# benjjneb/dada2

Measured on AMD Instinct MI355X. Metric: unique reads denoised/sec (dada() wall-clock), higher is better.
Workload: dtype int32 DP + f64 lambda/p-value

## Files before the change

dada2_amd/csrc/driver.cpp:

```cpp
#include <fcntl.h>
#include <sys/file.h>
#include <unistd.h>

#include <algorithm>
#include <atomic>
#include <chrono>
#include <condition_variable>
#include <exception>
#include <mutex>
#include <cmath>
#include <cstdarg>
#include <cstdio>
#include <cstring>
#include <ctime>
#include <memory>
#include <thread>
#include <unordered_map>

#include "engine.h"
#include "hostpar.h"
#include "knobs.h"
#include "ppois.h"

namespace d2 {
// ... 1544 lines not shown
    if (knobs().v2_summary) fprintf(stderr, "[v3] entry barrier failed after %ld blocks: continuing on the launch chains\n", v2_cons);
  }
  bool v3_block_ready() const { return *(volatile int32_t *)&v2_hblk.p[v2_cons % RING2].seq == (int32_t)(v2_cons + 1); }
  long v3_ended() const { return (long)*(volatile int32_t *)(v3_hflags.p + 16); }
  std::vector<EnqRec> v3_rec;
  void v3_enqueue(bool first) {
    const auto t_enq = clk::now();
    hipStream_t stq = s->stream;
    EnqRec rec{-1, -1, !first};
    if (!first) {
      rec.ev_screen = ev_begin(EV_SCREEN, profile_all, true);
      launch2_screen_multi(E2, stq);
      ev_end(rec.ev_screen);
      launch2_batch_lists(E2, stq);
      const NwBatch nb{&v2_ctl.p->nalign, v2_blistn.p, v2_blist.p, v2_ctl.p->acentre, &v2_ctl.p->abuf, E2.C.Npad, v2_bretry.p, v2_bretryn.p, v2_retrytot.p, &v2_ctl.p->fast_off};
      launch_gapless_batch(s->D, nb, ap, s->d_err.p, v2_lamB.p, v2_hamB.p, &v2_ctl.p->state, stq);
      rec.ev_nw = ev_begin(EV_NW, profile_all, true);
      launch_nw_ad(s->D, -1, nullptr, nullptr, nullptr, 0, nullptr, nullptr, ap, s->d_err.p, v2_lamB.p, v2_hamB.p, nullptr, 0, 0, nullptr, stq,
                   &v2_ctl.p->state, &nb);
      ev_end(rec.ev_nw);
    }
    const int ev = ev_begin(EV_TAIL, profile_all);
    Eng2 Ek = E2;
    if (!profile_all) Ek.ktime = nullptr;
    Ek.pf_plan = (v3_overlap && (active_runs(s->device).load() <= 1 || knobs().v3_overlap == 1)) ? 1 : 0;
    launch3_tail(Ek, v3_grid, first, (int)(v3_enq + 1), s->h_reads[bi[0].center], stq);
    ev_end(ev);
    v3_rec.push_back(rec);
    v3_enq++;
    st.ms_enqueue += ms_since(t_enq);
  }

  void v3_pf_enqueue(long k) {
    const auto t_enq = clk::now();
    hipStream_t st2 = s->cmp;
    Ctl2 *pc = v3_pfctl.p;
    *(volatile int32_t *)(v3_hflags.p + 40 + (k & 7)) = 0;
    launch2_pf_gate(E2P, (int)k, v3_hflags.p + 32, v3_hflags.p + 40 + (k & 7), st2);
    launch2_pf_tables(E2P, st2);
    int ev = ev_begin(EV_PF_SCREEN, profile_all, false, false, st2);
    launch2_screen_multi(E2P, st2);
    ev_end(ev);
    launch2_batch_lists(E2P, st2);
    const NwBatch nb{&pc->nalign, v3_pf_blistn.p, v3_pf_blist.p, pc->acentre, &pc->abuf, E2.C.Npad, v3_pf_bretry.p, v3_pf_bretryn.p, v2_retrytot.p, &pc->fast_off};
    launch_gapless_batch(S2, nb, ap, s->d_err.p, v2_lamB.p, v2_hamB.p, &pc->state, st2);
    ev = ev_begin(EV_PF_NW, profile_all, false, false, st2);
    launch_nw_ad(S2, -1, nullptr, nullptr, nullptr, 0, nullptr, nullptr, ap, s->d_err.p, v2_lamB.p, v2_hamB.p, nullptr, 0, 0, nullptr, st2,
                 &pc->state, &nb);
    ev_end(ev);
    launch2_pf_done(E2P, st2);
    D2_HIP(hipEventRecord(v3_pf_ev[k & 3], st2));
    v3_pf_launched = std::max(v3_pf_launched, k);
    v3_pf_chains++;
    st.ms_enqueue += ms_since(t_enq);
  }
  int v3_pf_gate_result(long k) const { return (int)*(volatile int32_t *)(v3_hflags.p + 40 + (k & 7)); }
  int32_t v3_pf_stat[4] = {0, 0, 0, 0};
  void v3_pf_totals() {
    PfSync ps;
    D2_HIP(hipMemcpy(&ps, v3_pfsync.p, sizeof ps, hipMemcpyDeviceToHost));
// ... 191 lines not shown
    if (lite) st.lite_chains++;
    v2_enqrec.push_back(rec);
    v2_enq++;
    st.ms_enqueue += ms_since(t_enq);
  }
  void v2_round_launches(int nlev, bool with_compare, bool store, EnqRec *recp, bool lite = false) {
    hipStream_t stq = s->stream;
    EnqRec rec{-1, -1, with_compare};
    const Eng2 &E2 = lite ? this->E2L : this->E2;
    if (with_compare && !lite) {
      rec.ev_screen = ev_begin(EV_SCREEN, profile_all, true);
      launch2_screen_multi(E2, stq);
      ev_end(rec.ev_screen);
      launch2_batch_lists(E2, stq);
      const NwBatch nb{&v2_ctl.p->nalign, v2_blistn.p, v2_blist.p, v2_ctl.p->acentre, &v2_ctl.p->abuf, E2.C.Npad, v2_bretry.p, v2_bretryn.p, v2_retrytot.p, &v2_ctl.p->fast_off};
      launch_gapless_batch(s->D, nb, ap, s->d_err.p, v2_lamB.p, v2_hamB.p, &v2_ctl.p->state, stq);
      rec.ev_nw = ev_begin(EV_NW, profile_all, true);
      launch_nw_ad(s->D, -1, nullptr, nullptr, nullptr, 0, nullptr, nullptr, ap, s->d_err.p, v2_lamB.p, v2_hamB.p, nullptr, 0, 0, nullptr, stq,
                   &v2_ctl.p->state, &nb);
      ev_end(rec.ev_nw);
    }
    int ev = ev_begin(EV_SHUFFLE, profile_all && nlev > 0);
    for (int l = 0; l < nlev; l++) launch2_shuffle(E2, l, store && l == 0, stq);
    ev_end(ev);
    ev = ev_begin(EV_PVAL, profile_all);
    launch2_eval(E2, nlev, s->h_reads[bi[0].center], stq);
    ev_end(ev);
    if (recp) *recp = rec;
  }

  const Round2Out &v2_wait_block() {
// ... 1380 lines not shown
```

dada2_amd/csrc/engine.h:

```cpp
#pragma once
#include <cstddef>
#include <cstdint>
#include <string>
#include <vector>

#include <hip/hip_runtime.h>

#include "../../include/dada2hip.h"

namespace d2 {

constexpr int KMER_SIZE = 5;
constexpr int NKMER = 1024;
constexpr int RANK_SAT = 63;
constexpr int MAX_SHUFFLE = 10;
constexpr int SEQLEN = 9999;
constexpr double TAIL_APPROX_CUTOFF = 1e-7;

enum : uint8_t { CLS_SKIP = 0, CLS_SHROUD = 1, CLS_GAPLESS = 2, CLS_NW = 3 };

struct DeviceError {
  int code;
  std::string msg;
};
// ... 167 lines not shown
               double *d_lambda, uint32_t *d_ham, uint16_t *d_view, int LV, int view_by_chunk, uint8_t *d_moves,
               int moves_stride, int32_t *d_nmoves, hipStream_t st, const int32_t *d_pair_centre = nullptr);

struct NwBatch {
  const int32_t *on;
  const int32_t *n;
  const int32_t *list;
  const int32_t *centre;
  const int32_t *bbuf;
  size_t stride;
  int32_t *retry_list = nullptr;
  int32_t *retry_n = nullptr;
  unsigned long long *fast_ctl = nullptr;
  const int32_t *fast_off = nullptr;
};
void launch_gapless_batch(const SampleDev &S, const NwBatch &b, const AlignParams &ap, const double *d_err, double *d_lambda,
                          uint32_t *d_ham, const int32_t *d_stop_dev, hipStream_t st);
void launch_nw_ad(const SampleDev &S, int centre, const int32_t *d_chunk_centre, const int32_t *d_work,
                  const int32_t *d_nwork, int nwork_host, const int32_t *d_gl_work, const int32_t *d_gl_nwork,
                  const AlignParams &ap, const double *d_err, double *d_lambda, uint32_t *d_ham, uint16_t *d_view, int LV,
                  int view_by_chunk, const int32_t *d_centre_dev, hipStream_t st, const int32_t *d_stop_dev = nullptr,
                  const NwBatch *batch = nullptr);
int nw_ad_apw(const SampleDev &S, const AlignParams &ap);
size_t nw_ad_lds_bytes(const SampleDev &S, const AlignParams &ap);
void launch_nw_ad_lr(const SampleDev &S, const int32_t *d_chunk_centre, const int32_t *d_work, int nwork, const AlignParams &ap,
                     const double *d_err, int allow_one_off, int max_shift, int32_t *d_out, hipStream_t st);
size_t nw_ad_lr_lds_bytes(const SampleDev &S, const AlignParams &ap);

bool nw_adw_ok(const SampleDev &S, const AlignParams &ap);
size_t nw_adw_ptr_words_per_wave(const SampleDev &S, const AlignParams &ap);
int nw_adw_waves(const SampleDev &S, const AlignParams &ap, int nwork);
size_t nw_adw_lds_bytes(const SampleDev &S, const AlignParams &ap);
// ... 307 lines not shown
```

dada2_amd/csrc/kernels.hip:

```cpp
#include <atomic>
#include <cstring>

#include "engine.h"
#include "gcn.h"
#include "knobs.h"
#include "rounds_common.h"
#include "ppois.h"

namespace d2 {

static std::atomic<uint64_t> g_ledger[LEDGER_WORDS];
void ledger_note(int bit) { g_ledger[bit >> 6].fetch_or((uint64_t)1 << (bit & 63), std::memory_order_relaxed); }
void ledger_read(uint64_t *out, bool clear) {
  for (int w = 0; w < LEDGER_WORDS; w++)
    out[w] = clear ? g_ledger[w].exchange(0, std::memory_order_relaxed) : g_ledger[w].load(std::memory_order_relaxed);
}
static std::atomic<int32_t> g_nw_trips{0};
void nw_trips_note(int trips) {
  int32_t cur = g_nw_trips.load(std::memory_order_relaxed);
  while (cur < trips && !g_nw_trips.compare_exchange_weak(cur, trips, std::memory_order_relaxed)) {}
}
int nw_trips_read(bool clear) { return clear ? g_nw_trips.exchange(0, std::memory_order_relaxed) : g_nw_trips.load(std::memory_order_relaxed); }

static __device__ __forceinline__ uint32_t base_at(const uint32_t *__restrict__ row, int p) {
// ... 302 lines not shown
    ham[r] = h;
  }
}

void launch_gapless(const SampleDev &S, int centre, const int32_t *d_chunk_centre, const int32_t *d_work,
                    const int32_t *d_nwork, int nwork_host, const AlignParams &ap, const double *d_err,
                    double *d_lambda, uint32_t *d_ham, uint16_t *d_view, int LV, int view_by_chunk, hipStream_t st) {
  int maxwork = d_nwork ? S.N : nwork_host;
  if (maxwork <= 0) return;
  int grid = std::min((maxwork + 255) / 256, 2048);
  ledger_note(LEDGER_GAPLESS);
  hipLaunchKernelGGL(k_gapless, dim3(grid), dim3(256), (size_t)16 * ap.ncol * sizeof(double), st, S, centre,
                     d_chunk_centre, d_work, d_nwork, nwork_host, ap, d_err, d_lambda, d_ham, d_view, LV, view_by_chunk);
}

__global__ __launch_bounds__(256) void k_gapless_batch(SampleDev S, NwBatch b, AlignParams ap, const double *__restrict__ err,
                                                       double *__restrict__ lam, uint32_t *__restrict__ ham, const int32_t *__restrict__ stop_dev) {
  if (stop_dev && *stop_dev != 0) return;
  const int nb = *b.on;
  if (nb <= 0) return;
  int wk[KB_MAX + 1];
  wk[0] = 0;
#pragma unroll
  for (int k = 0; k < KB_MAX; k++) wk[k + 1] = wk[k] + (k < nb ? (b.n[KB_MAX + k] + 63) / 64 : 0);
  if ((int)blockIdx.x * 4 >= wk[KB_MAX]) return;
  extern __shared__ double s_err[];
  for (int i = threadIdx.x; i < 16 * ap.ncol; i += blockDim.x) s_err[i] = err[i];
  __syncthreads();
  const int lane = threadIdx.x & 63, gwave = blockIdx.x * 4 + (threadIdx.x >> 6), nwaves = gridDim.x * 4;
  for (int w = gwave; w < wk[KB_MAX]; w += nwaves) {
    int k = 0, w0 = 0;
#pragma unroll
    for (int q = 1; q < KB_MAX; q++) if (w >= wk[q]) { k = q; w0 = wk[q]; }
    const int idx = (w - w0) * 64 + lane;
    if (idx >= b.n[KB_MAX + k]) continue;
    const int r = b.list[(size_t)(KB_MAX + k) * b.stride + idx], c = b.centre[k];
    const uint32_t *crow = S.seq2 + (size_t)c * S.W2, *rrow = S.seq2 + (size_t)r * S.W2;
    const uint8_t *qrow = S.qual + (size_t)r * S.LQ;
    const int L1 = S.len[c], L2 = S.len[r];
    double l = 1.0;
    uint32_t h = 0, cw = 0, rw = 0, qw = 0;
    for (int p = 0; p < L2; p++) {
      if ((p & 15) == 0) { rw = rrow[p >> 4]; cw = p < L1 ? crow[p >> 4] : 0; }
      if ((p & 3) == 0) qw = *(const uint32_t *)(qrow + p);
      const uint32_t rb = (rw >> ((p & 15) << 1)) & 3u, q = ap.use_quals ? ((qw >> ((p & 3) << 3)) & 255u) : 0u;
      uint32_t t = 5u * rb;
      if (p < L1) {
        const uint32_t cb = (cw >> ((p & 15) << 1)) & 3u;
        t = 4u * cb + rb;
        h += (cb != rb);
      }
      l = l * s_err[t * ap.ncol + q];
    }
    const size_t o = ((size_t)*b.bbuf * KB_MAX + k) * b.stride + r;
    lam[o] = l;
    ham[o] = h;
  }
}
void launch_gapless_batch(const SampleDev &S, const NwBatch &b, const AlignParams &ap, const double *d_err, double *d_lambda,
                          uint32_t *d_ham, const int32_t *d_stop_dev, hipStream_t st) {
  const int grid = std::min((S.N + 255) / 256 + KB_MAX, 2048);
  ledger_note(LEDGER_GAPLESS + 1);
  hipLaunchKernelGGL(k_gapless_batch, dim3(grid), dim3(256), (size_t)16 * ap.ncol * sizeof(double), st, S, b, ap, d_err, d_lambda, d_ham,
                     d_stop_dev);
}

struct NwArgs {
  SampleDev S;
  int centre;
  const int32_t *centre_dev;
  const int32_t *chunk_centre;
  const int32_t *pair_centre;
  const int32_t *work;
  const int32_t *nwork_dev;
  int nwork_host;
  AlignParams ap;
  const double *err;
  uint32_t *ptr_scr;
  uint32_t *t_scr;
// ... 4 lines not shown
  uint16_t *view;
  int LV;
  int view_by_chunk;
  uint8_t *moves;
  int moves_stride;
  int32_t *nmoves;
  const int32_t *stop_dev;
  int32_t *lr_out;
  int lr_one_off, lr_max_shift;
  const int32_t *batch_on;
  const int32_t *batch_n;
  const int32_t *batch_list;
  const int32_t *batch_centre;
  const int32_t *batch_bbuf;
  size_t batch_stride;
  int32_t *retry_list;
  int32_t *retry_n;
  unsigned long long *fast_ctl;
  const int32_t *fast_off;
  const int32_t *alt_list;
  const int32_t *alt_n;
};

template <int NPW>
static __device__ __forceinline__ void nw_traceback_lambda(const NwArgs &a, const double *s_err, int lane, int idx,
                                                           bool active, int r, int c, int L1, int L2, int lband,
                                                           const uint32_t *ptr, uint32_t *tsc, int npw_rt, int chunk) {
  const SampleDev &S = a.S;
  const size_t vr = a.view_by_chunk ? (size_t)chunk : (size_t)r;
  const uint32_t *crow = S.seq2 + (size_t)c * S.W2, *rrow = S.seq2 + (size_t)r * S.W2;
// ... 461 lines not shown
__global__ __launch_bounds__(256, 4) void k_nw_ad(NwArgs a, const int32_t *__restrict__ gl_work, const int32_t *__restrict__ gl_nwork_dev,
                                               AdGeom G) {
  static_assert(!FAST || (DEF && !LR && !HOMO), "the pointer-free pass exists for the default scores of the denoising path");
  constexpr int APW = 64 / GL;
  extern __shared__ __attribute__((aligned(16))) double s_dyn[];
  double *s_err = s_dyn;
  const int nerr = 16 * a.ap.ncol;
  const bool batch = a.batch_on != nullptr;
  int bk[KB_MAX + 1];
  {
    if (a.stop_dev && *a.stop_dev != 0) return;
    bk[0] = 0;
    if (batch) {
      const int nb = *a.batch_on;
      if (nb <= 0) return;
      if (a.fast_off) {
        const bool off = *a.fast_off != 0;
        if (FAST) {
          if (off) return;
          if (blockIdx.x == 0 && threadIdx.x == 0) {
            unsigned long long tot = 0;
            for (int k = 0; k < KB_MAX; k++) tot += k < nb ? (unsigned long long)a.batch_n[k] : 0ull;
            atomicAdd(&a.fast_ctl[1], tot);
          }
        } else if (off && a.alt_list) { a.batch_list = a.alt_list; a.batch_n = a.alt_n; }
      }
#pragma unroll
      for (int k = 0; k < KB_MAX; k++) bk[k + 1] = bk[k] + (k < nb ? (a.batch_n[k] + 4 * APW - 1) / (4 * APW) : 0);
      if ((int)blockIdx.x >= bk[KB_MAX]) return;
    } else {
      const int n_all = (a.nwork_dev ? *a.nwork_dev : a.nwork_host) + (gl_work ? *gl_nwork_dev : 0);
      if ((int)blockIdx.x * 4 * APW >= n_all) return;
      if (a.centre_dev && *a.centre_dev < 0) return;
    }
  }
  for (int i = threadIdx.x; i < nerr; i += blockDim.x) s_err[i] = a.err[i];
  const int wib = threadIdx.x >> 6, lane = threadIdx.x & 63;
  const bool ghost = lane / GL >= APW;
  const int al = ghost ? APW - 1 : lane / GL, g = ghost ? GL : lane % GL;
  uint8_t *blk0 = (uint8_t *)(s_dyn + nerr);
// ... 12 lines not shown
      for (int p = threadIdx.x; p < Lc; p += 256) cwd[p] = ad_base_word<HOMO>(S.seq2 + (size_t)cv * S.W2, Lc, p);
    }
  }
  __syncthreads();
  const int gwave = blockIdx.x * 4 + wib;
  uint32_t *pg = S.ad_ptr + (size_t)gwave * S.ad_wpw;
  int n_nw = batch ? 0 : (a.nwork_dev ? *a.nwork_dev : a.nwork_host);
  const int n_gl = batch ? 0 : (gl_work ? *gl_nwork_dev : 0);
  int nwork = n_nw + n_gl;
  const int SENT = a.ap.sentinel, MATCH = a.ap.match, MISMATCH = a.ap.mismatch, GAP = a.ap.gap, B = a.ap.band, HGAP = a.ap.homo_gap;
  const int centre_v = batch ? 0 : (a.centre_dev ? *a.centre_dev : a.centre);
  if (centre_v < 0 && !a.chunk_centre) return;
  const int32_t *wl = a.work, *gll = gl_work;
  size_t out_off = 0;
  int kcur = -1;
  for (int it = blockIdx.x;; it += gridDim.x) {
    int chunk, c;
    if (batch) {
      if (it >= bk[KB_MAX]) break;
      int k = 0, b0 = 0;
#pragma unroll
      for (int q = 1; q < KB_MAX; q++) if (it >= bk[q]) { k = q; b0 = bk[q]; }
      c = a.batch_centre[k];
      if (k != kcur) {
        __syncthreads();
        const int Lc = S.len[c];
        for (int p = threadIdx.x; p < Lc; p += 256) cwd[p] = ad_base_word<HOMO>(S.seq2 + (size_t)c * S.W2, Lc, p);
        __syncthreads();
        kcur = k;
        wl = a.batch_list + (size_t)k * a.batch_stride; gll = a.batch_list + (size_t)(KB_MAX + k) * a.batch_stride;
        n_nw = a.batch_n[k]; nwork = n_nw;
// ... 20 lines not shown
      for (int p = g; p < L2; p += GL) rwd[p] = ad_base_word<HOMO>(S.seq2 + (size_t)r * S.W2, L2, p);
    if (LR && !ghost)
      for (int w = g; w < 3 * G.bmw; w += GL) bm[w] = 0;
    int ecol = 0;
    const uint8_t *qrow = S.qual + (size_t)r * S.LQ;
    const size_t vr = a.view_by_chunk ? (size_t)chunk : (size_t)r;
    if (a.view && active && !ghost)
      for (int p = g; p < L1; p += GL) a.view[vr * a.LV + p] = 0;
    int Tmax = T;
#pragma unroll
    for (int o = 32; o >= 1; o >>= 1) Tmax = max(Tmax, __shfl_xor(Tmax, o, 64));
    const int dbg = a.moves_stride;
    Tmax = gcn_readfirstlane(Tmax);
    const int org = (EDGE ? 0 : 2) + (lband & 1), lbo = lband + org;
    uint32_t acc0 = ~0u, acc1 = ~0u, ep0 = 3u, ep1 = 3u;
    if (Tmax >= 0 && !(dbg & 1)) {
      int d0 = SENT, d1 = SENT;
      uint32_t pw = 0;
      int i = (lbo >> 1) - g, j = -i;
      uint32_t cb = cwd[i - 1], rb = rwd[j - 1];
      const bool g_first = g == 0, g_last = ghost || g == GL - 1;
      const bool kok0 = !ghost && 2 * g >= org && 2 * g < W + org, kok1 = !ghost && 2 * g + 1 >= org && 2 * g + 1 < W + org;
      constexpr int KUP = ADK_GAP + (int)AD_UP - (int)AD_DIAG, KLEFT = ADK_GAP + (int)AD_LEFT - (int)AD_DIAG;
      const int gs0 = DEF ? (kok0 ? KUP : ADK_BIG) : (kok0 ? GAP : AD_OOB), gs1 = DEF ? (kok1 ? KLEFT : ADK_BIG) : (kok1 ? GAP : AD_OOB);
      const int gn0 = DEF ? ((EDGE && g_first) || !kok0 ? ADK_BIG : KLEFT) : gs0, gn1 = DEF ? ((EDGE && g_last) || !kok1 ? ADK_BIG : KUP) : gs1;
      if (DEF) { d0 = ADK_BIG + (int)AD_DIAG; d1 = ADK_BIG + (int)AD_DIAG; }
      int tA = (lband > rband ? lband : rband) + 2, tB = min(2 * L1 - lband, 2 * L2 - rband);
      if (T < 0) { tA = 0; tB = 0x3FFFFFFF; }
#pragma unroll
      for (int o = 32; o >= 1; o >>= 1) { tA = max(tA, __shfl_xor(tA, o, 64)); tB = min(tB, __shfl_xor(tB, o, 64)); }
      tA = gcn_readfirstlane(tA);
      tB = gcn_readfirstlane(tB);
#define AD_FLUSH(TT) { if (!FAST) { pg[(size_t)((TT) >> 4) * 64 + lane] = pw; pw = 0; } }
#define AD_STEP(PARV, LEANV, VNEXT, FS, KOK, GS)                                                                                   \
  {                                                                                                                             \
    if (FAST) ad_step_k<GL, PARV, LEANV, EDGE, true>(d0, d1, i, j, cb, rb, (PARV) ? acc1 : acc0, (VNEXT), (FS), g_first, g_last, (KOK), (GS), (PARV) ? gn1 : gn0, L1, L2, (PARV) ? &ep1 : &ep0); \
    else if (DEF) ad_step_k<GL, PARV, LEANV, EDGE>(d0, d1, i, j, cb, rb, pw, (VNEXT), (FS), g_first, g_last, (KOK), (GS), (PARV) ? gn1 : gn0, L1, L2); \
    else ad_step<GL, PARV, DEF, LEANV, EDGE, HOMO>(d0, d1, i, j, cb, rb, pw, (VNEXT), (FS), g_first, g_last, (KOK), (GS), L1, L2, SENT, MATCH, MISMATCH, GAP, HGAP); \
  }
#define AD_FULL_STEP(TT)                                                                                                        \
  {                                                                                                                             \
    if (((TT) & 1) == 0) AD_STEP(0, false, rwd[j], ((TT) & 15) << 1, kok0, gs0)                                                 \
    else AD_STEP(1, false, cwd[i], ((TT) & 15) << 1, kok1, gs1)                                                                 \
    if (((TT) & 15) == 15) AD_FLUSH(TT)                                                                                         \
  }
#define AD_LEAN_PAIR(TT)                                                                                                        \
  {                                                                                                                             \
    AD_STEP(0, true, rwd[j], ((TT) & 15) << 1, kok0, gs0)                                                                       \
    AD_STEP(1, true, cwd[i], (((TT) + 1) & 15) << 1, kok1, gs1)                                                                 \
    if ((((TT) + 1) & 15) == 15) AD_FLUSH((TT) + 1)                                                                             \
  }
// ... 6 lines not shown
        __builtin_memcpy(rwv, rwd + j, 32);
        __builtin_memcpy(cwv, cwd + i, 32);
#pragma unroll
        for (int u = 0; u < 8; u++) {
          AD_STEP(0, true, rwv[u], 4 * u, kok0, gs0)
          AD_STEP(1, true, cwv[u], 4 * u + 2, kok1, gs1)
        }
        AD_FLUSH(t)
      }
      for (; t + 2 <= tB && t + 1 <= Tmax; t += 2) AD_LEAN_PAIR(t)
      for (; t <= Tmax; t++) AD_FULL_STEP(t)
#undef AD_LEAN_PAIR
#undef AD_FULL_STEP
#undef AD_STEP
#undef AD_FLUSH
      if (!FAST && ((t - 1) & 15) != 15) pg[(size_t)((t - 1) >> 4) * 64 + lane] = pw >> (2 * (15 - ((t - 1) & 15)));
    }
    int fres = 0, fk = 0, fm = 0, fdir = -1;
    if (FAST) {
      fk = L2 - L1 + lbo;
      if (T < 0) fres = 2;
      for (int itw = 0; itw <= 2 * GL + 1; itw++) {
        if (__all(fres != 0)) break;
        const bool inband = fk >= org && fk < W + org;
        const int src = al * GL + (inband ? (fk >> 1) : 0);
        const uint32_t e0 = (uint32_t)__shfl((int)ep0, src, 64), e1 = (uint32_t)__shfl((int)ep1, src, 64);
        const uint32_t a0 = (uint32_t)__shfl((int)acc0, src, 64), a1 = (uint32_t)__shfl((int)acc1, src, 64);
        if (fres != 0) continue;
        const uint32_t pe = (fk & 1) ? e1 : e0, whole = (((fk & 1) ? a1 : a0) >> 1) & 1u;
        if (!inband || pe > AD_DIAG) fres = 2;
        else if (pe == AD_DIAG) fres = whole ? 1 : 2;
        else if (fdir < 0 || (int)pe == fdir) { fdir = (int)pe; fm++; fk += pe == AD_UP ? 1 : -1; }
        else fres = 2;
      }
      if (fres == 0) fres = 2;
    }
    int ti = L1, tj = L2;
    bool done = !active || (dbg & 2);
    uint32_t h = 0;
    int guard = L1 + L2 + 2;
    while (true) {
      int nruns = 0;
      uint32_t last = 0;
      auto push = [&](int lo, int n, int dl) {
        if (last) {
          const int llo = last & 4095, ln = (last >> 12) & 4095, ldl = (int)(last >> 24);
          if (ldl == dl && lo + n == llo) { last = (uint32_t)lo | ((uint32_t)(ln + n) << 12) | ((uint32_t)dl << 24); return; }
          runs[nruns++] = last;
        }
        last = (uint32_t)lo | ((uint32_t)n << 12) | ((uint32_t)dl << 24);
      };
      const bool lead = g == 0 && !ghost;
      if (lead && !done && gapless) {
        const int n = L1 < L2 ? L1 : L2;
        runs[nruns++] = 0u | ((uint32_t)n << 12) | (128u << 24);
        if (L2 > n) runs[nruns++] = (uint32_t)n | ((uint32_t)(L2 - n) << 12) | (255u << 24);
        done = true;
      }
      if (FAST && lead && !done) {
        if (fres == 1) {
          const int dd = fk - lbo;
          const int n = dd >= 0 ? min(L1, L2 - dd) : min(L1 + dd, L2);
          if (fdir == (int)AD_LEFT && fm > 0) runs[nruns++] = (uint32_t)(L2 - fm) | ((uint32_t)fm << 12) | (255u << 24);
          if (n > 0) runs[nruns++] = (uint32_t)(dd >= 0 ? dd : 0) | ((uint32_t)n << 12) | ((uint32_t)(128 - dd) << 24);
          if (dd > 0) runs[nruns++] = 0u | ((uint32_t)dd << 12) | (255u << 24);
        } else if (active && !gapless) {
          const int q = atomicAdd(&a.retry_n[kcur], 1);
          a.retry_list[(size_t)kcur * a.batch_stride + q] = r;
          if (a.fast_ctl) atomicAdd(&a.fast_ctl[0], 1ull);
        }
        done = true; ti = 0; tj = 0;
      }
      const int gl0 = al * GL;
      if (!FAST)
      for (;;) {
        const bool act = lead && !done && (ti > 0 || tj > 0) && nruns < AD_RCAP - 2 && guard > 0;
        if (!__any(act)) break;
        bool gapmove = false;
        const int gact = __shfl((int)act, gl0, 64);
        const int tt = __shfl(ti + tj, gl0, 64), col = __shfl((tj - ti + lbo) >> 1, gl0, 64);
        const int f0 = tt & 15, widx = (tt >> 4) - g;
        uint32_t word = 0xAAAAAAAAu;
        if (gact && !ghost && widx >= 0) word = pg[(size_t)widx * 64 + gl0 + col];
        const int ftop = g == 0 ? f0 : 14 + (f0 & 1);
        const uint32_t x = word ^ 0xAAAAAAAAu;
        uint32_t nz = (x | (x >> 1)) & 0x55555555u;
        nz &= (f0 & 1) ? 0x44444444u : 0x11111111u;
        nz &= (ftop == 15) ? 0xFFFFFFFFu : ((1u << ((ftop + 1) << 1)) - 1u);
        const bool st = nz != 0;
// ... 83 lines not shown
      if (__all(done)) break;
    }
    if (LR) {
      gcn_wave_sync();
      if (g == 0 && !ghost && active)
        bimera_lr_bits(bm, bm + G.bmw, bm + 2 * G.bmw, ecol, a.lr_one_off, a.lr_max_shift, a.lr_out + (size_t)idx * 5);
      continue;
    }
    if (g == 0 && !ghost) runs[0] = 0;
    gcn_wave_sync();
    if (!ghost && h) atomicAdd(&runs[0], h);
    gcn_wave_sync();
    h = runs[0];
    const long long fid = ((long long)it * 4 + wib) * APW + al;
    const bool offload = S.ad_foff != nullptr && fid < (long long)S.ad_fcap && !(dbg & 8);
    if (FAST && fres != 1) continue;
    if (offload) {
      if (active && !ghost) {
        uint16_t *fo = S.ad_foff + (size_t)fid * S.ad_fstride;
        for (int pj = g; pj < L2; pj += GL) fo[pj] = (uint16_t)rwd[pj];
        if (g == 0) {
          AdDesc d;
          d.dest = (long long)(out_off + r); d.L2 = L2; d.pad = 0;
          S.ad_desc[fid] = d;
          a.ham[out_off + r] = h;
        }
      }
    } else
    if (g == 0 && active && !(dbg & 8)) {
      const char *eb = (const char *)s_err;
      auto fetch8 = [&](int pj, double (&f)[8]) __attribute__((always_inline)) {
// ... 15 lines not shown
          for (int k = 0; k < 8; k++) f[k] = n[k];
        }
#pragma unroll
        for (int k = 0; k < 8; k++) l = l * f[k];
      }
      for (; pj < L2; pj++) l = l * *(const double *)(eb + rwd[pj]);
      a.lam[out_off + r] = l;
      a.ham[out_off + r] = h;
    }
  }
}

__global__ __launch_bounds__(256) void k_ad_product(const uint16_t *__restrict__ foff, int stride, AdDesc *__restrict__ desc, int nscan,
                                                    const double *__restrict__ err, int nerr, double *__restrict__ lam,
                                                    const int32_t *__restrict__ stop_dev, const int32_t *__restrict__ batch_on,
                                                    const int32_t *__restrict__ batch_n, int slots_per_slice,
                                                    const int32_t *__restrict__ fast_off = nullptr, const int32_t *__restrict__ alt_n = nullptr) {
  extern __shared__ double s_err[];
  if (stop_dev && *stop_dev != 0) return;
  if (fast_off && alt_n && *fast_off != 0) batch_n = alt_n;
  if (batch_on) {
    const int nb = *batch_on;
    if (nb <= 0) return;
    int slices = 0;
    for (int k = 0; k < KB_MAX; k++) slices += k < nb ? (batch_n[k] + slots_per_slice - 1) / slots_per_slice : 0;
    nscan = min(nscan, slices * slots_per_slice);
  }
  if ((int)(blockIdx.x * blockDim.x) >= nscan) return;
  for (int i = threadIdx.x; i < nerr; i += blockDim.x) s_err[i] = err[i];
  __syncthreads();
  const char *eb = (const char *)s_err;
  for (int id = blockIdx.x * blockDim.x + threadIdx.x; id < nscan; id += gridDim.x * blockDim.x) {
    const AdDesc d = desc[id];
    if (d.dest < 0) continue;
    desc[id].dest = -1;
// ... 26 lines not shown
  a.S = S; a.centre = centre; a.chunk_centre = d_chunk_centre; a.work = d_work; a.nwork_dev = d_nwork;
  a.nwork_host = nwork_host; a.ap = ap; a.err = d_err; a.lam = d_lambda; a.ham = d_ham;
  a.view = d_view; a.LV = LV; a.view_by_chunk = view_by_chunk; a.centre_dev = d_centre_dev; a.stop_dev = d_stop_dev;
#ifdef DADA2HIP_PROFILING
  a.moves_stride = knobs().ad_debug;
#endif
  if (batch) {
    a.batch_on = batch->on; a.batch_n = batch->n; a.batch_list = batch->list; a.batch_centre = batch->centre; a.batch_bbuf = batch->bbuf;
    a.batch_stride = batch->stride;
  }
  const AdGeom G = ad_geom(ap.band, S.maxlen, S.minlen, d_chunk_centre ? 0 : 1);
  const size_t lds = (size_t)16 * ap.ncol * 8 + (size_t)G.block_bytes;
  int waves = (std::max(maxwork, 1) + G.APW - 1) / G.APW;
  if (d_gl_work || batch) waves = (S.N + G.APW - 1) / G.APW;
  int grid = std::max(1, std::min((waves + 3) / 4, std::min(256 * 8, S.ad_waves / 4)));
  const bool homo = ap.endsfree && ap.homo_gap != ap.gap;
  const bool def = !homo && ap.match == 5 && ap.mismatch == -4 && ap.gap == -8 && ap.sentinel == -32760;
  const bool fast = batch && def && batch->retry_list && batch->retry_n && batch->fast_off && knobs().ad_fast != 0 && a.moves_stride == 0;
  auto set_lds = [&](const void *fn, std::atomic<size_t> (&done)[64]) {
    int dev_ = 0;
    (void)hipGetDevice(&dev_);
    std::atomic<size_t> &d = done[dev_ & 63];
    if (lds > d.load(std::memory_order_acquire)) {
      (void)hipFuncSetAttribute(fn, hipFuncAttributeMaxDynamicSharedMemorySize, (int)lds);
      d.store(lds, std::memory_order_release);
    }
  };
#define D2_LAUNCH_AD(GLV, DEFV, EDGEV, HOMOV, FASTV)                                                                     \
  do {                                                                                                                   \
    static std::atomic<size_t> attr_set[64];                                                                             \
    set_lds((const void *)k_nw_ad<GLV, DEFV, EDGEV, false, HOMOV, FASTV>, attr_set);                                     \
    ledger_note(LEDGER_AD + 8 * (GLV == 21 ? 0 : GLV == 32 ? 1 : 2) + 4 * (EDGEV ? 1 : 0) + (FASTV ? 3 : HOMOV ? 2 : DEFV ? 0 : 1)); \
    hipLaunchKernelGGL((k_nw_ad<GLV, DEFV, EDGEV, false, HOMOV, FASTV>), dim3(grid), dim3(256), lds, st, a, d_gl_work, d_gl_nwork, G);  \
  } while (0)
#define D2_LAUNCH_AD2(GLV, FASTV)                                                                                        \
  do {                                                                                                                   \
    if (FASTV) { if (G.edge) D2_LAUNCH_AD(GLV, true, true, false, FASTV); else D2_LAUNCH_AD(GLV, true, false, false, FASTV); } \
    else if (homo) { if (G.edge) D2_LAUNCH_AD(GLV, false, true, true, false); else D2_LAUNCH_AD(GLV, false, false, true, false); } \
    else if (def) { if (G.edge) D2_LAUNCH_AD(GLV, true, true, false, false); else D2_LAUNCH_AD(GLV, true, false, false, false); } \
    else { if (G.edge) D2_LAUNCH_AD(GLV, false, true, false, false); else D2_LAUNCH_AD(GLV, false, false, false, false); }   \
  } while (0)
  auto product = [&](const int32_t *list_n, const int32_t *foff = nullptr, const int32_t *alt_n = nullptr) {
    if (!(S.ad_foff && a.moves_stride == 0)) return;
    const int nerr = 16 * ap.ncol;
    long long bound = batch ? (long long)S.ad_fcap : (long long)((maxwork + (d_gl_work ? S.N : 0) + 4 * G.APW - 1) / (4 * G.APW) + 1) * 4 * G.APW;
    const int nscan = (int)std::min<long long>(bound, S.ad_fcap);
    const int pgrid = std::max(1, std::min((nscan + 255) / 256, 2048));
    hipLaunchKernelGGL(k_ad_product, dim3(pgrid), dim3(256), (size_t)nerr * 8, st, (const uint16_t *)S.ad_foff, (int)S.ad_fstride, S.ad_desc, nscan, d_err, nerr,
                       d_lambda, d_stop_dev, batch ? batch->on : nullptr, list_n, 4 * G.APW, foff, alt_n);
  };
  if (fast) {
    a.retry_list = batch->retry_list; a.retry_n = batch->retry_n; a.fast_ctl = batch->fast_ctl; a.fast_off = batch->fast_off;
    if (G.GL == 21) D2_LAUNCH_AD2(21, true);
    else if (G.GL == 32) D2_LAUNCH_AD2(32, true);
    else D2_LAUNCH_AD2(64, true);
    product(batch->n);
    a.alt_list = a.batch_list; a.alt_n = a.batch_n;
    a.batch_list = batch->retry_list; a.batch_n = batch->retry_n;
    a.retry_list = nullptr; a.retry_n = nullptr;
  }
  if (G.GL == 21) D2_LAUNCH_AD2(21, false);
  else if (G.GL == 32) D2_LAUNCH_AD2(32, false);
  else D2_LAUNCH_AD2(64, false);
#undef D2_LAUNCH_AD2
#undef D2_LAUNCH_AD
  if (fast) product(batch->retry_n, batch->fast_off, batch->n);
  else product(batch ? batch->n : nullptr);
}

void launch_nw_ad_lr(const SampleDev &S, const int32_t *d_chunk_centre, const int32_t *d_work, int nwork, const AlignParams &ap,
                     const double *d_err, int allow_one_off, int max_shift, int32_t *d_out, hipStream_t st) {
  if (nwork <= 0) return;
  NwArgs a;
  memset(&a, 0, sizeof a);
  a.S = S; a.chunk_centre = d_chunk_centre; a.work = d_work; a.nwork_host = nwork; a.ap = ap; a.err = d_err;
  a.lr_out = d_out; a.lr_one_off = allow_one_off; a.lr_max_shift = max_shift;
  const AdGeom G = ad_geom(ap.band, S.maxlen, S.minlen, 0, 1);
  const size_t lds = (size_t)16 * ap.ncol * 8 + (size_t)G.block_bytes;
  const int waves = (nwork + G.APW - 1) / G.APW;
  const int grid = std::max(1, std::min((waves + 3) / 4, std::min(256 * 8, S.ad_waves / 4)));
  const bool def = ap.match == 5 && ap.mismatch == -4 && ap.gap == -8 && ap.sentinel == -32760;
#define D2_LAUNCH_LR(GLV, DEFV, EDGEV)                                                                                   \
// ... 1144 lines not shown
```

Baseline: 7.380 million.

## Fuse gapless batch into NW kernel blocks and resweep fast-path failures in-kernel

Removes the separate gapless-batch kernel launch and runs its work in extra blocks appended to the k_nw_ad grid, selected by block index. The FAST variant now resweeps failing alignments in place with full pointer recording instead of pushing them to a retry list. The product kernel is also launched once at the end instead of twice. This cuts kernel launches and queue gaps in the compare chain, at the cost of a larger grid, mixed block roles, and more register and code pressure in the NW kernel.

```diff
diff --git a/dada2_amd/csrc/driver.cpp b/dada2_amd/csrc/driver.cpp
--- a/dada2_amd/csrc/driver.cpp
+++ b/dada2_amd/csrc/driver.cpp
@@ -1582,7 +1582,6 @@
       ev_end(rec.ev_screen);
       launch2_batch_lists(E2, stq);
       const NwBatch nb{&v2_ctl.p->nalign, v2_blistn.p, v2_blist.p, v2_ctl.p->acentre, &v2_ctl.p->abuf, E2.C.Npad, v2_bretry.p, v2_bretryn.p, v2_retrytot.p, &v2_ctl.p->fast_off};
-      launch_gapless_batch(s->D, nb, ap, s->d_err.p, v2_lamB.p, v2_hamB.p, &v2_ctl.p->state, stq);
       rec.ev_nw = ev_begin(EV_NW, profile_all, true);
       launch_nw_ad(s->D, -1, nullptr, nullptr, nullptr, 0, nullptr, nullptr, ap, s->d_err.p, v2_lamB.p, v2_hamB.p, nullptr, 0, 0, nullptr, stq,
                    &v2_ctl.p->state, &nb);
@@ -1611,7 +1610,6 @@
     ev_end(ev);
     launch2_batch_lists(E2P, st2);
     const NwBatch nb{&pc->nalign, v3_pf_blistn.p, v3_pf_blist.p, pc->acentre, &pc->abuf, E2.C.Npad, v3_pf_bretry.p, v3_pf_bretryn.p, v2_retrytot.p, &pc->fast_off};
-    launch_gapless_batch(S2, nb, ap, s->d_err.p, v2_lamB.p, v2_hamB.p, &pc->state, st2);
     ev = ev_begin(EV_PF_NW, profile_all, false, false, st2);
     launch_nw_ad(S2, -1, nullptr, nullptr, nullptr, 0, nullptr, nullptr, ap, s->d_err.p, v2_lamB.p, v2_hamB.p, nullptr, 0, 0, nullptr, st2,
                  &pc->state, &nb);
@@ -1833,7 +1831,6 @@
       ev_end(rec.ev_screen);
       launch2_batch_lists(E2, stq);
       const NwBatch nb{&v2_ctl.p->nalign, v2_blistn.p, v2_blist.p, v2_ctl.p->acentre, &v2_ctl.p->abuf, E2.C.Npad, v2_bretry.p, v2_bretryn.p, v2_retrytot.p, &v2_ctl.p->fast_off};
-      launch_gapless_batch(s->D, nb, ap, s->d_err.p, v2_lamB.p, v2_hamB.p, &v2_ctl.p->state, stq);
       rec.ev_nw = ev_begin(EV_NW, profile_all, true);
       launch_nw_ad(s->D, -1, nullptr, nullptr, nullptr, 0, nullptr, nullptr, ap, s->d_err.p, v2_lamB.p, v2_hamB.p, nullptr, 0, 0, nullptr, stq,
                    &v2_ctl.p->state, &nb);
diff --git a/dada2_amd/csrc/engine.h b/dada2_amd/csrc/engine.h
--- a/dada2_amd/csrc/engine.h
+++ b/dada2_amd/csrc/engine.h
@@ -205,8 +205,6 @@
   unsigned long long *fast_ctl = nullptr;
   const int32_t *fast_off = nullptr;
 };
-void launch_gapless_batch(const SampleDev &S, const NwBatch &b, const AlignParams &ap, const double *d_err, double *d_lambda,
-                          uint32_t *d_ham, const int32_t *d_stop_dev, hipStream_t st);
 void launch_nw_ad(const SampleDev &S, int centre, const int32_t *d_chunk_centre, const int32_t *d_work,
                   const int32_t *d_nwork, int nwork_host, const int32_t *d_gl_work, const int32_t *d_gl_nwork,
                   const AlignParams &ap, const double *d_err, double *d_lambda, uint32_t *d_ham, uint16_t *d_view, int LV,
diff --git a/dada2_amd/csrc/kernels.hip b/dada2_amd/csrc/kernels.hip
--- a/dada2_amd/csrc/kernels.hip
+++ b/dada2_amd/csrc/kernels.hip
@@ -1,5 +1,6 @@
 #include <atomic>
 #include <cstring>
+#include <type_traits>
 
 #include "engine.h"
 #include "gcn.h"
@@ -340,27 +341,26 @@
                      d_chunk_centre, d_work, d_nwork, nwork_host, ap, d_err, d_lambda, d_ham, d_view, LV, view_by_chunk);
 }
 
-__global__ __launch_bounds__(256) void k_gapless_batch(SampleDev S, NwBatch b, AlignParams ap, const double *__restrict__ err,
-                                                       double *__restrict__ lam, uint32_t *__restrict__ ham, const int32_t *__restrict__ stop_dev) {
-  if (stop_dev && *stop_dev != 0) return;
-  const int nb = *b.on;
-  if (nb <= 0) return;
+static __device__ __forceinline__ void gapless_batch_block(const SampleDev &S, int nb, const int32_t *__restrict__ bn,
+                                                           const int32_t *__restrict__ blist, size_t stride,
+                                                           const int32_t *__restrict__ bcentre, const int32_t *__restrict__ bbuf,
+                                                           const AlignParams &ap, const double *__restrict__ err, double *s_err,
+                                                           double *__restrict__ lam, uint32_t *__restrict__ ham, int gb, int ngb) {
   int wk[KB_MAX + 1];
   wk[0] = 0;
 #pragma unroll
-  for (int k = 0; k < KB_MAX; k++) wk[k + 1] = wk[k] + (k < nb ? (b.n[KB_MAX + k] + 63) / 64 : 0);
-  if ((int)blockIdx.x * 4 >= wk[KB_MAX]) return;
-  extern __shared__ double s_err[];
+  for (int k = 0; k < KB_MAX; k++) wk[k + 1] = wk[k] + (k < nb ? (bn[KB_MAX + k] + 63) / 64 : 0);
+  if (gb * 4 >= wk[KB_MAX]) return;
   for (int i = threadIdx.x; i < 16 * ap.ncol; i += blockDim.x) s_err[i] = err[i];
   __syncthreads();
-  const int lane = threadIdx.x & 63, gwave = blockIdx.x * 4 + (threadIdx.x >> 6), nwaves = gridDim.x * 4;
+  const int lane = threadIdx.x & 63, gwave = gb * 4 + (threadIdx.x >> 6), nwaves = ngb * 4;
   for (int w = gwave; w < wk[KB_MAX]; w += nwaves) {
     int k = 0, w0 = 0;
 #pragma unroll
     for (int q = 1; q < KB_MAX; q++) if (w >= wk[q]) { k = q; w0 = wk[q]; }
     const int idx = (w - w0) * 64 + lane;
-    if (idx >= b.n[KB_MAX + k]) continue;
-    const int r = b.list[(size_t)(KB_MAX + k) * b.stride + idx], c = b.centre[k];
+    if (idx >= bn[KB_MAX + k]) continue;
+    const int r = blist[(size_t)(KB_MAX + k) * stride + idx], c = bcentre[k];
     const uint32_t *crow = S.seq2 + (size_t)c * S.W2, *rrow = S.seq2 + (size_t)r * S.W2;
     const uint8_t *qrow = S.qual + (size_t)r * S.LQ;
     const int L1 = S.len[c], L2 = S.len[r];
@@ -378,17 +378,10 @@
       }
       l = l * s_err[t * ap.ncol + q];
     }
-    const size_t o = ((size_t)*b.bbuf * KB_MAX + k) * b.stride + r;
+    const size_t o = ((size_t)*bbuf * KB_MAX + k) * stride + r;
     lam[o] = l;
     ham[o] = h;
   }
-}
-void launch_gapless_batch(const SampleDev &S, const NwBatch &b, const AlignParams &ap, const double *d_err, double *d_lambda,
-                          uint32_t *d_ham, const int32_t *d_stop_dev, hipStream_t st) {
-  const int grid = std::min((S.N + 255) / 256 + KB_MAX, 2048);
-  ledger_note(LEDGER_GAPLESS + 1);
-  hipLaunchKernelGGL(k_gapless_batch, dim3(grid), dim3(256), (size_t)16 * ap.ncol * sizeof(double), st, S, b, ap, d_err, d_lambda, d_ham,
-                     d_stop_dev);
 }
 
 struct NwArgs {
@@ -423,6 +416,7 @@
   const int32_t *batch_centre;
   const int32_t *batch_bbuf;
   size_t batch_stride;
+  int nw_blocks, gl_mode;
   int32_t *retry_list;
   int32_t *retry_n;
   unsigned long long *fast_ctl;
@@ -914,6 +908,7 @@
     if (batch) {
       const int nb = *a.batch_on;
       if (nb <= 0) return;
+      bool gl_on = a.gl_mode == 1;
       if (a.fast_off) {
         const bool off = *a.fast_off != 0;
         if (FAST) {
@@ -923,7 +918,16 @@
             for (int k = 0; k < KB_MAX; k++) tot += k < nb ? (unsigned long long)a.batch_n[k] : 0ull;
             atomicAdd(&a.fast_ctl[1], tot);
           }
-        } else if (off && a.alt_list) { a.batch_list = a.alt_list; a.batch_n = a.alt_n; }
+        } else {
+          if (off && a.alt_list) { a.batch_list = a.alt_list; a.batch_n = a.alt_n; }
+          if (a.gl_mode == 2) gl_on = off;
+        }
+      }
+      if ((int)blockIdx.x >= a.nw_blocks) {
+        if (gl_on)
+          gapless_batch_block(a.S, nb, a.batch_n, a.batch_list, a.batch_stride, a.batch_centre, a.batch_bbuf, a.ap, a.err, s_err, a.lam, a.ham,
+                              (int)blockIdx.x - a.nw_blocks, (int)gridDim.x - a.nw_blocks);
+        return;
       }
 #pragma unroll
       for (int k = 0; k < KB_MAX; k++) bk[k + 1] = bk[k] + (k < nb ? (a.batch_n[k] + 4 * APW - 1) / (4 * APW) : 0);
@@ -966,7 +970,8 @@
   const int32_t *wl = a.work, *gll = gl_work;
   size_t out_off = 0;
   int kcur = -1;
-  for (int it = blockIdx.x;; it += gridDim.x) {
+  const int it_stride = batch ? a.nw_blocks : (int)gridDim.x;
+  for (int it = blockIdx.x;; it += it_stride) {
     int chunk, c;
     if (batch) {
       if (it >= bk[KB_MAX]) break;
@@ -1017,7 +1022,8 @@
     Tmax = gcn_readfirstlane(Tmax);
     const int org = (EDGE ? 0 : 2) + (lband & 1), lbo = lband + org;
     uint32_t acc0 = ~0u, acc1 = ~0u, ep0 = 3u, ep1 = 3u;
-    if (Tmax >= 0 && !(dbg & 1)) {
+    auto sweep = [&](auto pf_tag, const int T, const int Tmax) __attribute__((always_inline)) {
+      constexpr bool PF = decltype(pf_tag)::value;
       int d0 = SENT, d1 = SENT;
       uint32_t pw = 0;
       int i = (lbo >> 1) - g, j = -i;
@@ -1034,10 +1040,10 @@
       for (int o = 32; o >= 1; o >>= 1) { tA = max(tA, __shfl_xor(tA, o, 64)); tB = min(tB, __shfl_xor(tB, o, 64)); }
       tA = gcn_readfirstlane(tA);
       tB = gcn_readfirstlane(tB);
-#define AD_FLUSH(TT) { if (!FAST) { pg[(size_t)((TT) >> 4) * 64 + lane] = pw; pw = 0; } }
+#define AD_FLUSH(TT) { if (!PF) { pg[(size_t)((TT) >> 4) * 64 + lane] = pw; pw = 0; } }
 #define AD_STEP(PARV, LEANV, VNEXT, FS, KOK, GS)                                                                                   \
   {                                                                                                                             \
-    if (FAST) ad_step_k<GL, PARV, LEANV, EDGE, true>(d0, d1, i, j, cb, rb, (PARV) ? acc1 : acc0, (VNEXT), (FS), g_first, g_last, (KOK), (GS), (PARV) ? gn1 : gn0, L1, L2, (PARV) ? &ep1 : &ep0); \
+    if (PF) ad_step_k<GL, PARV, LEANV, EDGE, true>(d0, d1, i, j, cb, rb, (PARV) ? acc1 : acc0, (VNEXT), (FS), g_first, g_last, (KOK), (GS), (PARV) ? gn1 : gn0, L1, L2, (PARV) ? &ep1 : &ep0); \
     else if (DEF) ad_step_k<GL, PARV, LEANV, EDGE>(d0, d1, i, j, cb, rb, pw, (VNEXT), (FS), g_first, g_last, (KOK), (GS), (PARV) ? gn1 : gn0, L1, L2); \
     else ad_step<GL, PARV, DEF, LEANV, EDGE, HOMO>(d0, d1, i, j, cb, rb, pw, (VNEXT), (FS), g_first, g_last, (KOK), (GS), L1, L2, SENT, MATCH, MISMATCH, GAP, HGAP); \
   }
@@ -1074,8 +1080,9 @@
 #undef AD_FULL_STEP
 #undef AD_STEP
 #undef AD_FLUSH
-      if (!FAST && ((t - 1) & 15) != 15) pg[(size_t)((t - 1) >> 4) * 64 + lane] = pw >> (2 * (15 - ((t - 1) & 15)));
-    }
+      if (!PF && ((t - 1) & 15) != 15) pg[(size_t)((t - 1) >> 4) * 64 + lane] = pw >> (2 * (15 - ((t - 1) & 15)));
+    };
+    if (Tmax >= 0 && !(dbg & 1)) sweep(std::integral_constant<bool, FAST>{}, T, Tmax);
     int fres = 0, fk = 0, fm = 0, fdir = -1;
     if (FAST) {
       fk = L2 - L1 + lbo;
@@ -1094,6 +1101,20 @@
         else fres = 2;
       }
       if (fres == 0) fres = 2;
+    }
+    bool resweep = false;
+    if (FAST) {
+      const bool need = T >= 0 && fres != 1;
+      const unsigned long long nb_ = __ballot(need && g == 0 && !ghost);
+      resweep = nb_ != 0ull;
+      if (resweep) {
+        if (lane == 0 && a.fast_ctl) atomicAdd(&a.fast_ctl[0], (unsigned long long)__popcll(nb_));
+        const int T2 = need ? T : -1;
+        int T2max = T2;
+#pragma unroll
+        for (int o = 32; o >= 1; o >>= 1) T2max = max(T2max, __shfl_xor(T2max, o, 64));
+        sweep(std::false_type{}, T2, gcn_readfirstlane(T2max));
+      }
     }
     int ti = L1, tj = L2;
     bool done = !active || (dbg & 2);
@@ -1117,22 +1138,16 @@
         if (L2 > n) runs[nruns++] = (uint32_t)n | ((uint32_t)(L2 - n) << 12) | (255u << 24);
         done = true;
       }
-      if (FAST && lead && !done) {
-        if (fres == 1) {
-          const int dd = fk - lbo;
-          const int n = dd >= 0 ? min(L1, L2 - dd) : min(L1 + dd, L2);
-          if (fdir == (int)AD_LEFT && fm > 0) runs[nruns++] = (uint32_t)(L2 - fm) | ((uint32_t)fm << 12) | (255u << 24);
-          if (n > 0) runs[nruns++] = (uint32_t)(dd >= 0 ? dd : 0) | ((uint32_t)n << 12) | ((uint32_t)(128 - dd) << 24);
-          if (dd > 0) runs[nruns++] = 0u | ((uint32_t)dd << 12) | (255u << 24);
-        } else if (active && !gapless) {
-          const int q = atomicAdd(&a.retry_n[kcur], 1);
-          a.retry_list[(size_t)kcur * a.batch_stride + q] = r;
-          if (a.fast_ctl) atomicAdd(&a.fast_ctl[0], 1ull);
-        }
+      if (FAST && lead && !done && fres == 1) {
+        const int dd = fk - lbo;
+        const int n = dd >= 0 ? min(L1, L2 - dd) : min(L1 + dd, L2);
+        if (fdir == (int)AD_LEFT && fm > 0) runs[nruns++] = (uint32_t)(L2 - fm) | ((uint32_t)fm << 12) | (255u << 24);
+        if (n > 0) runs[nruns++] = (uint32_t)(dd >= 0 ? dd : 0) | ((uint32_t)n << 12) | ((uint32_t)(128 - dd) << 24);
+        if (dd > 0) runs[nruns++] = 0u | ((uint32_t)dd << 12) | (255u << 24);
         done = true; ti = 0; tj = 0;
       }
       const int gl0 = al * GL;
-      if (!FAST)
+      if (!FAST || resweep)
       for (;;) {
         const bool act = lead && !done && (ti > 0 || tj > 0) && nruns < AD_RCAP - 2 && guard > 0;
         if (!__any(act)) break;
@@ -1246,7 +1261,6 @@
     h = runs[0];
     const long long fid = ((long long)it * 4 + wib) * APW + al;
     const bool offload = S.ad_foff != nullptr && fid < (long long)S.ad_fcap && !(dbg & 8);
-    if (FAST && fres != 1) continue;
     if (offload) {
       if (active && !ghost) {
         uint16_t *fo = S.ad_foff + (size_t)fid * S.ad_fstride;
@@ -1292,11 +1306,9 @@
 __global__ __launch_bounds__(256) void k_ad_product(const uint16_t *__restrict__ foff, int stride, AdDesc *__restrict__ desc, int nscan,
                                                     const double *__restrict__ err, int nerr, double *__restrict__ lam,
                                                     const int32_t *__restrict__ stop_dev, const int32_t *__restrict__ batch_on,
-                                                    const int32_t *__restrict__ batch_n, int slots_per_slice,
-                                                    const int32_t *__restrict__ fast_off = nullptr, const int32_t *__restrict__ alt_n = nullptr) {
+                                                    const int32_t *__restrict__ batch_n, int slots_per_slice) {
   extern __shared__ double s_err[];
   if (stop_dev && *stop_dev != 0) return;
-  if (fast_off && alt_n && *fast_off != 0) batch_n = alt_n;
   if (batch_on) {
     const int nb = *batch_on;
     if (nb <= 0) return;
@@ -1353,6 +1365,9 @@
   int waves = (std::max(maxwork, 1) + G.APW - 1) / G.APW;
   if (d_gl_work || batch) waves = (S.N + G.APW - 1) / G.APW;
   int grid = std::max(1, std::min((waves + 3) / 4, std::min(256 * 8, S.ad_waves / 4)));
+  const int ggrid = batch ? std::min((S.N + 255) / 256 + KB_MAX, 2048) : 0;
+  a.nw_blocks = grid; a.gl_mode = batch ? 1 : 0;
+  if (batch) ledger_note(LEDGER_GAPLESS + 1);
   const bool homo = ap.endsfree && ap.homo_gap != ap.gap;
   const bool def = !homo && ap.match == 5 && ap.mismatch == -4 && ap.gap == -8 && ap.sentinel == -32760;
   const bool fast = batch && def && batch->retry_list && batch->retry_n && batch->fast_off && knobs().ad_fast != 0 && a.moves_stride == 0;
@@ -1370,7 +1385,7 @@
     static std::atomic<size_t> attr_set[64];                                                                             \
     set_lds((const void *)k_nw_ad<GLV, DEFV, EDGEV, false, HOMOV, FASTV>, attr_set);                                     \
     ledger_note(LEDGER_AD + 8 * (GLV == 21 ? 0 : GLV == 32 ? 1 : 2) + 4 * (EDGEV ? 1 : 0) + (FASTV ? 3 : HOMOV ? 2 : DEFV ? 0 : 1)); \
-    hipLaunchKernelGGL((k_nw_ad<GLV, DEFV, EDGEV, false, HOMOV, FASTV>), dim3(grid), dim3(256), lds, st, a, d_gl_work, d_gl_nwork, G);  \
+    hipLaunchKernelGGL((k_nw_ad<GLV, DEFV, EDGEV, false, HOMOV, FASTV>), dim3(grid + ggrid), dim3(256), lds, st, a, d_gl_work, d_gl_nwork, G);  \
   } while (0)
 #define D2_LAUNCH_AD2(GLV, FASTV)                                                                                        \
   do {                                                                                                                   \
@@ -1379,32 +1394,31 @@
     else if (def) { if (G.edge) D2_LAUNCH_AD(GLV, true, true, false, false); else D2_LAUNCH_AD(GLV, true, false, false, false); } \
     else { if (G.edge) D2_LAUNCH_AD(GLV, false, true, false, false); else D2_LAUNCH_AD(GLV, false, false, false, false); }   \
   } while (0)
-  auto product = [&](const int32_t *list_n, const int32_t *foff = nullptr, const int32_t *alt_n = nullptr) {
+  auto product = [&](const int32_t *list_n) {
     if (!(S.ad_foff && a.moves_stride == 0)) return;
     const int nerr = 16 * ap.ncol;
     long long bound = batch ? (long long)S.ad_fcap : (long long)((maxwork + (d_gl_work ? S.N : 0) + 4 * G.APW - 1) / (4 * G.APW) + 1) * 4 * G.APW;
     const int nscan = (int)std::min<long long>(bound, S.ad_fcap);
     const int pgrid = std::max(1, std::min((nscan + 255) / 256, 2048));
     hipLaunchKernelGGL(k_ad_product, dim3(pgrid), dim3(256), (size_t)nerr * 8, st, (const uint16_t *)S.ad_foff, (int)S.ad_fstride, S.ad_desc, nscan, d_err, nerr,
-                       d_lambda, d_stop_dev, batch ? batch->on : nullptr, list_n, 4 * G.APW, foff, alt_n);
+                       d_lambda, d_stop_dev, batch ? batch->on : nullptr, list_n, 4 * G.APW);
   };
   if (fast) {
     a.retry_list = batch->retry_list; a.retry_n = batch->retry_n; a.fast_ctl = batch->fast_ctl; a.fast_off = batch->fast_off;
     if (G.GL == 21) D2_LAUNCH_AD2(21, true);
     else if (G.GL == 32) D2_LAUNCH_AD2(32, true);
     else D2_LAUNCH_AD2(64, true);
-    product(batch->n);
     a.alt_list = a.batch_list; a.alt_n = a.batch_n;
     a.batch_list = batch->retry_list; a.batch_n = batch->retry_n;
     a.retry_list = nullptr; a.retry_n = nullptr;
+    a.gl_mode = 2;
   }
   if (G.GL == 21) D2_LAUNCH_AD2(21, false);
   else if (G.GL == 32) D2_LAUNCH_AD2(32, false);
   else D2_LAUNCH_AD2(64, false);
 #undef D2_LAUNCH_AD2
 #undef D2_LAUNCH_AD
-  if (fast) product(batch->retry_n, batch->fast_off, batch->n);
-  else product(batch ? batch->n : nullptr);
+  product(batch ? batch->n : nullptr);
 }
 
 void launch_nw_ad_lr(const SampleDev &S, const int32_t *d_chunk_centre, const int32_t *d_work, int nwork, const AlignParams &ap,
diff --git a/profiles/compare_chain.py b/profiles/compare_chain.py
--- /dev/null
+++ b/profiles/compare_chain.py
@@ -0,0 +1,73 @@
+#!/usr/bin/env python3
+import sqlite3
+import sys
+from collections import Counter, defaultdict
+
+
+def short(n):
+    n = n.replace("d2::", "").replace("void ", "")
+    base = n.split("(")[0]
+    if base.startswith("k_nw_ad<"):
+        args = base[len("k_nw_ad<"):].rstrip(">").split(", ")
+        return "k_nw_ad<FAST>" if len(args) >= 6 and args[5] == "true" else "k_nw_ad<full>"
+    return base.split("<")[0]
+
+
+def pct(v, q):
+    v = sorted(v)
+    return v[min(len(v) - 1, max(0, int(round(q * (len(v) - 1)))))]
+
+
+def chains(path):
+    db = sqlite3.connect(path)
+    rows = list(db.execute("select name, stream, start, end from kernels order by start"))
+    by_stream = defaultdict(list)
+    for n, s, a, b in rows:
+        by_stream[s].append((short(n), a, b))
+    out = []
+    for s, ks in by_stream.items():
+        if not any(k[0] == "k2_pf_done" for k in ks):
+            continue
+        cur = None
+        for k in ks:
+            if k[0] == "k2_pf_gate":
+                cur = []
+            elif cur is not None:
+                cur.append(k)
+                if k[0] == "k2_pf_done":
+                    out.append(cur)
+                    cur = None
+    return out
+
+
+def report(path):
+    work = [c for c in chains(path) if any(k[0].startswith("k2_screen_multi") and k[2] - k[1] >= 8000 for k in c)]
+    print(f"## {path}: {len(work)} working prefetch compares")
+    if not work:
+        return
+    span = [(c[-1][2] - c[0][1]) / 1e3 for c in work]
+    busy = [sum(k[2] - k[1] for k in c) / 1e3 for c in work]
+    print("chain first kernel start -> k2_pf_done end, us: median %.1f, 10-90 %% %.1f-%.1f" % (pct(span, .5), pct(span, .1), pct(span, .9)))
+    print("  of which kernels: median %.1f; gaps: median %.1f" % (pct(busy, .5), pct([a - b for a, b in zip(span, busy)], .5)))
+    per = defaultdict(list)
+    nlaunch = Counter()
+    for c in work:
+        seen = Counter()
+        for n, a, b in c:
+            seen[n] += 1
+            per[n if seen[n] == 1 else f"{n} #{seen[n]}"].append((b - a) / 1e3)
+        for n, v in seen.items():
+            nlaunch[(n, v)] += 1
+    print("| kernel | compares with it | median us | 10-90 % |")
+    print("|---|---|---|---|")
+    for n, v in per.items():
+        print("| `%s` | %d | %.1f | %.1f-%.1f |" % (n, len(v), pct(v, .5), pct(v, .1), pct(v, .9)))
+    print("launches per compare:", ", ".join("%s x%d in %d" % (n, v, c) for (n, v), c in sorted(nlaunch.items())))
+    full = [(k[2] - k[1]) / 1e3 for c in work for k in c if k[0] == "k_nw_ad<full>"]
+    if full:
+        print("k_nw_ad<full> launches in working compares: %d, longest %.1f us" % (len(full), max(full)))
+    print()
+
+
+for p in sys.argv[1:]:
+    report(p)
```

New measurement: 7.549 million (median of 5 runs). Within noise of the previous version (+2.3%).
